# UCSD-Comp-Imaging/Nerf-Simple

Measured on AMD Instinct MI355X. Metric: ray-samples/sec at 800x800x128, higher is better.
Workload: dtype f16

## Files before the change

nerf-simple_amd/csrc/dw_gemm.hip:

```cpp
#include "nerf_device.h"
#include "launchers.h"

using namespace nerf_layout;

typedef __bf16 bf16x4 __attribute__((ext_vector_type(4)));

namespace {

constexpr int MAXD = 16;
struct GemmDesc {
    const __bf16* A;
    const __bf16* B;
    float* C;
    int lda, ldb, ldc;
    int M, N;
    int r0, Mv, Nv;
    int wg0, wgs;
    float* bias;
};
struct GemmTable {
    GemmDesc d[MAXD];
    int n;
    long long P;
};

constexpr int SLAB = 32;
static_assert(SLAB == 32, "the slab loop is written for two k-steps");
static_assert(ACT_TILE_PTS % SLAB == 0 && ACT_TILE_PTS * 16 == 4096, "a slab never straddles activation blocks");
constexpr int ROWB = 512;
constexpr int OPB = SLAB * ROWB;
constexpr int KSTEP = 16 * ROWB;
constexpr int SLOTB = 2 * OPB;
constexpr int RING = 4;
constexpr int LDS_BYTES = RING * SLOTB;
constexpr int DMA_PER_SLAB = 2 * SLAB / 2 / 8;

struct Frag { bf16x4 lo, hi; };
template <int KOFF>
__device__ __forceinline__ void read_frag_tr(Frag& f, unsigned addr_lo, unsigned addr_hi) {
    asm volatile("ds_read_b64_tr_b16 %0, %2 offset:%4\n\tds_read_b64_tr_b16 %1, %3 offset:%4"
                 : "=&v"(f.lo), "=&v"(f.hi) : "v"(addr_lo), "v"(addr_hi), "n"(KOFF));
}
__device__ __forceinline__ void frags_landed(Frag (&a)[4], Frag (&b)[2]) {
    asm volatile("s_waitcnt lgkmcnt(0)"
                 : "+v"(a[0].lo), "+v"(a[0].hi), "+v"(a[1].lo), "+v"(a[1].hi), "+v"(a[2].lo), "+v"(a[2].hi),
                   "+v"(a[3].lo), "+v"(a[3].hi), "+v"(b[0].lo), "+v"(b[0].hi), "+v"(b[1].lo), "+v"(b[1].hi));
}
__device__ __forceinline__ bf16x8 whole(const Frag& f) {
    return bf16x8{f.lo[0], f.lo[1], f.lo[2], f.lo[3], f.hi[0], f.hi[1], f.hi[2], f.hi[3]};
}

__global__ __launch_bounds__(512, 2) void dw_gemm_kernel(GemmTable tab) {
    extern __shared__ __attribute__((aligned(16))) char smem[];
    int di = 0;
    while (di + 1 < tab.n && (int)blockIdx.x >= tab.d[di + 1].wg0) ++di;
    const GemmDesc d = tab.d[di];
    const int slice = blockIdx.x - d.wg0;
    const long long nslab = (tab.P + SLAB - 1) / SLAB;
    const long long s_begin = nslab * slice / d.wgs, s_end = nslab * (slice + 1) / d.wgs;

    const int tid = threadIdx.x, lane = tid & 63;
    const int wave = __builtin_amdgcn_readfirstlane(tid >> 6);
    const int wm = wave >> 2, wn = wave & 3;
    const int m0 = 128 * wm, n0 = 64 * wn;

    const bool pieceA = wave < 4;
    const int pld = pieceA ? d.lda : d.ldb;
    const bool pblk = pld == 0;
    const __bf16* pbase = pieceA ? d.A : d.B;
    const int pwidth = pieceA ? d.M : d.N;
    const long long row_begin = s_begin * SLAB;
    const long long row_end = s_end * SLAB < tab.P ? s_end * SLAB : tab.P;
    const long long slice_rows = row_end > row_begin ? row_end - row_begin : 0;
    const long long slice_blocks = (row_end + ACT_TILE_PTS - 1) / ACT_TILE_PTS - row_begin / ACT_TILE_PTS;
    const __amdgpu_buffer_rsrc_t rs = pblk
        ? __builtin_amdgcn_make_buffer_rsrc(const_cast<char*>(reinterpret_cast<const char*>(pbase))
                                                + (row_begin / ACT_TILE_PTS) * ACT_BLOCK_BYTES,
                                            0, (int)(slice_rows > 0 ? slice_blocks * ACT_BLOCK_BYTES : 0), 0x00020000)
        : __builtin_amdgcn_make_buffer_rsrc(const_cast<__bf16*>(pbase + row_begin * pld), 0,
                                            (int)(slice_rows * pld * 2), 0x00020000);
    constexpr unsigned OUTSIDE = 0xffffffffu;
    unsigned voff[DMA_PER_SLAB];
    unsigned ldst[DMA_PER_SLAB];
    int vrow[DMA_PER_SLAB];
#pragma unroll
    for (int k = 0; k < DMA_PER_SLAB; ++k) {
        const int piece = wave * DMA_PER_SLAB + k, pi = piece & 15;
        ldst[k] = (piece >> 4) * OPB + pi * 1024;
        if (pblk) {
            const int c = 4 * (pi & 7) + (lane >> 4);
            vrow[k] = 16 * (pi >> 3) + ((lane & 15) ^ ((lane >> 4) << 2));
            voff[k] = c * 8 < pwidth ? (unsigned)(c * (ACT_TILE_PTS * 16) + vrow[k] * 16) : OUTSIDE;
        } else {
            vrow[k] = 2 * pi + (lane >> 5);
            const int cg = (lane & 31) ^ ((vrow[k] & 3) << 2);
            voff[k] = cg * 8 < pwidth ? (unsigned)(vrow[k] * pld * 2 + cg * 16) : OUTSIDE;
        }
    }
    auto issue_slab = [&](int it, int slot) {
        const long long p0 = row_begin + (long long)it * SLAB;
        unsigned vadd;
        int rows_left = SLAB;
        if (pblk) {
            vadd = (unsigned)((p0 / ACT_TILE_PTS - row_begin / ACT_TILE_PTS) * ACT_BLOCK_BYTES + (p0 % ACT_TILE_PTS) * 16);
            rows_left = tab.P - p0 < SLAB ? (int)(tab.P - p0) : SLAB;
        } else {
            vadd = (unsigned)it * (unsigned)(SLAB * pld * 2);
        }
#pragma unroll
        for (int k = 0; k < DMA_PER_SLAB; ++k) {
            lds_void* dst = reinterpret_cast<lds_void*>(reinterpret_cast<lds_char*>(0) + slot * SLOTB + ldst[k]);
            const unsigned off = (voff[k] == OUTSIDE || vrow[k] >= rows_left) ? OUTSIDE : voff[k] + vadd;
            __builtin_amdgcn_raw_ptr_buffer_load_lds(rs, dst, 16, off, 0, 0, 2);
        }
    };

    const int grp = lane >> 4, q = (lane & 15) >> 2, pp = lane & 3, h = lane >> 5;
    const int cl = 2 * (grp & 1) + (pp >> 1);
    auto frag_addr = [&](bool blocked, int t, int second) -> unsigned {
        const int r = 8 * h + q + 4 * second;
        if (blocked) return (4 * t + cl) * 256 + ((r ^ (cl << 2)) * 16) + 8 * (pp & 1);
        return r * ROWB + ((((4 * t + cl) ^ ((r & 3) << 2))) * 16) + 8 * (pp & 1);
    };
    unsigned aoff[4][2], boff[2][2];
#pragma unroll
    for (int i = 0; i < 4; ++i)
#pragma unroll
        for (int e = 0; e < 2; ++e) aoff[i][e] = frag_addr(d.lda == 0, m0 / 32 + i, e);
#pragma unroll
    for (int j = 0; j < 2; ++j)
#pragma unroll
        for (int e = 0; e < 2; ++e) boff[j][e] = OPB + frag_addr(d.ldb == 0, n0 / 32 + j, e);

    f32x16 acc[4][2];
#pragma unroll
    for (int i = 0; i < 4; ++i)
#pragma unroll
        for (int j = 0; j < 2; ++j)
#pragma unroll
            for (int r = 0; r < 16; ++r) acc[i][j][r] = 0.f;
    const bool active = m0 < d.M && n0 < d.N;
    float bsum[8] = {0.f, 0.f, 0.f, 0.f, 0.f, 0.f, 0.f, 0.f};
    const int brow = tid & 15, bchunk = tid >> 4;
    const unsigned baddr = bchunk * 256 + ((brow ^ ((bchunk & 3) << 2)) * 16);

#pragma unroll
    for (int k = 0; k < RING - 1; ++k)
        if (s_begin + k < s_end) issue_slab(k, k);
    Frag a0[4], b0[2], a1[4], b1[2];
    auto read_k0 = [&](unsigned base) {
#pragma unroll
        for (int i = 0; i < 4; ++i) read_frag_tr<0>(a0[i], base + aoff[i][0], base + aoff[i][1]);
#pragma unroll
        for (int j = 0; j < 2; ++j) read_frag_tr<0>(b0[j], base + boff[j][0], base + boff[j][1]);
    };
    if (s_begin < s_end) {
        const long long n = s_end - s_begin;
        if (n >= 3) asm volatile("s_waitcnt vmcnt(8)" ::: "memory");
        else if (n == 2) asm volatile("s_waitcnt vmcnt(4)" ::: "memory");
        else asm volatile("s_waitcnt vmcnt(0)" ::: "memory");
        __builtin_amdgcn_s_barrier();
        if (active) read_k0(0);
    }
    for (long long s = s_begin; s < s_end; ++s) {
        const int it = (int)(s - s_begin), slot = it & (RING - 1);
        const long long left = s_end - s;
        const unsigned base = slot * SLOTB;
        if (active) {
            frags_landed(a0, b0);
#pragma unroll
            for (int i = 0; i < 4; ++i) read_frag_tr<KSTEP>(a1[i], base + aoff[i][0], base + aoff[i][1]);
#pragma unroll
            for (int j = 0; j < 2; ++j) read_frag_tr<KSTEP>(b1[j], base + boff[j][0], base + boff[j][1]);
            __builtin_amdgcn_sched_barrier(0);
#pragma unroll
            for (int i = 0; i < 4; ++i)
#pragma unroll
                for (int j = 0; j < 2; ++j)
                    acc[i][j] = __builtin_amdgcn_mfma_f32_32x32x16_bf16(whole(a0[i]), whole(b0[j]), acc[i][j], 0, 0, 0);
            __builtin_amdgcn_sched_barrier(0);
        }
        if (left >= 2) {
            if (left >= 3) asm volatile("s_waitcnt vmcnt(4)" ::: "memory");
            else asm volatile("s_waitcnt vmcnt(0)" ::: "memory");
            __builtin_amdgcn_s_barrier();
            if (s + RING - 1 < s_end) issue_slab(it + RING - 1, (it + RING - 1) & (RING - 1));
        }
        if (active) {
            frags_landed(a1, b1);
            if (left >= 2) read_k0(((it + 1) & (RING - 1)) * SLOTB);
            __builtin_amdgcn_sched_barrier(0);
#pragma unroll
            for (int i = 0; i < 4; ++i)
#pragma unroll
                for (int j = 0; j < 2; ++j)
                    acc[i][j] = __builtin_amdgcn_mfma_f32_32x32x16_bf16(whole(a1[i]), whole(b1[j]), acc[i][j], 0, 0, 0);
        }
        if (d.bias && bchunk * 8 < d.M) {
#pragma unroll
            for (int ks = 0; ks < SLAB / 16; ++ks) {
                const bf16x8 v = *reinterpret_cast<const __attribute__((address_space(3))) bf16x8*>(
                    reinterpret_cast<lds_char*>(0) + base + ks * KSTEP + baddr);
#pragma unroll
                for (int k = 0; k < 8; ++k) bsum[k] += (float)v[k];
            }
        }
    }
    __syncthreads();
    if (d.bias && bchunk * 8 < d.M && s_begin < s_end) {
        float* red = reinterpret_cast<float*>(smem);
#pragma unroll
        for (int k = 0; k < 8; ++k) red[(brow * 32 + bchunk) * 8 + k] = bsum[k];
    }
    __syncthreads();
    if (d.bias && s_begin < s_end && tid < d.M) {
        const int ch = tid >> 3, k = tid & 7;
        float v = 0.f;
        for (int r = 0; r < 16; ++r) v += reinterpret_cast<float*>(smem)[(r * 32 + ch) * 8 + k];
        atomicAdd(d.bias + tid, v);
    }
    if (active && s_begin < s_end) {
#pragma unroll
        for (int i = 0; i < 4; ++i)
#pragma unroll
            for (int j = 0; j < 2; ++j)
#pragma unroll
                for (int r = 0; r < 16; ++r) {
                    const int row = m0 + 32 * i + (r & 3) + 8 * (r >> 2) + 4 * h - d.r0;
                    const int col = n0 + 32 * j + (lane & 31);
                    if (row >= 0 && row < d.Mv && col < d.Nv)
                        atomicAdd(d.C + (long long)row * d.ldc + col, acc[i][j][r]);
                }
    }
}

__global__ __launch_bounds__(256) void pack_draw_kernel(const float* __restrict__ d_raw, __bf16* __restrict__ dsr,
                                                        long long P, float* __restrict__ g_rgb_b,
                                                        float* __restrict__ g_sig_b) {
    __shared__ float red[4][4];
    f32x4 s = {0.f, 0.f, 0.f, 0.f};
    const __bf16 z = (__bf16)0.f;
    for (long long p = blockIdx.x * (long long)blockDim.x + threadIdx.x; p < P; p += (long long)gridDim.x * blockDim.x) {
        const f32x4 d = *reinterpret_cast<const f32x4*>(d_raw + p * 4);
        s += d;
        bf16x8* o = reinterpret_cast<bf16x8*>(dsr + p * 32);
        o[0] = bf16x8{(__bf16)d[0], (__bf16)d[1], (__bf16)d[2], (__bf16)d[3], z, z, z, z};
        o[1] = bf16x8{z, z, z, z, z, z, z, z};
        o[2] = o[1];
        o[3] = o[1];
    }
#pragma unroll
    for (int k = 0; k < 4; ++k) {
        float v = s[k];
#pragma unroll
        for (int off = 32; off >= 1; off >>= 1) v += __shfl_xor(v, off);
        if ((threadIdx.x & 63) == 0) red[threadIdx.x >> 6][k] = v;
    }
    __syncthreads();
    if (threadIdx.x < 4) {
        const float v = red[0][threadIdx.x] + red[1][threadIdx.x] + red[2][threadIdx.x] + red[3][threadIdx.x];
        atomicAdd(threadIdx.x < 3 ? g_rgb_b + threadIdx.x : g_sig_b, v);
    }
}

__global__ __launch_bounds__(256) void zero_f32_kernel(float* __restrict__ p, long long n) {
    const long long i = (blockIdx.x * (long long)blockDim.x + threadIdx.x) * 4;
    if (i + 3 < n) *reinterpret_cast<f32x4*>(p + i) = f32x4{0.f, 0.f, 0.f, 0.f};
    else for (long long k = i; k < n; ++k) p[k] = 0.f;
}

}

extern "C" int nerf_amd_launch_param_gradients_begin(const float* d_raw, void* scratch, float* grads, long long P,
                                                     hipStream_t stream) {
    (void)hipGetLastError();
    static_assert(PARAM_COUNT % 4 == 0, "16-byte zero fill");
    hipLaunchKernelGGL(zero_f32_kernel, dim3((PARAM_COUNT / 4 + 255) / 256), dim3(256), 0, stream, grads,
                       (long long)PARAM_COUNT);
    hipError_t e = hipGetLastError();
    if (e != hipSuccess) return (int)e;
    if (P <= 0) return 0;
    hipLaunchKernelGGL(pack_draw_kernel, dim3(512), dim3(256), 0, stream, d_raw, reinterpret_cast<__bf16*>(scratch), P,
                       grads + OFF_C1_B, grads + OFF_SIG_B);
    return (int)hipGetLastError();
}

extern "C" int nerf_amd_launch_param_gradients_finish(const void* acts_v, const void* dys_v, const void* posx64_v,
                                                      const void* posd32_v, const void* scratch, float* grads,
                                                      long long P, int bucket, hipStream_t stream) {
    (void)hipGetLastError();
    hipError_t e = hipSuccess;
    if (P <= 0) return 0;
    const __bf16* acts = reinterpret_cast<const __bf16*>(acts_v);
    const __bf16* dys = reinterpret_cast<const __bf16*>(dys_v);
    const __bf16* posx = reinterpret_cast<const __bf16*>(posx64_v);
    const __bf16* posd = reinterpret_cast<const __bf16*>(posd32_v);
    const __bf16* dsr = reinterpret_cast<const __bf16*>(scratch);
    auto act = [&](int L) { return acts + act_offset_bytes(L, P) / 2; };
    auto dy = [&](int L) { return dys + act_offset_bytes(L, P) / 2; };
    constexpr int BLK = 0;

    GemmTable t{};
    t.P = P;
    int n = 0;
    auto add = [&](const __bf16* A, int lda, int M, const __bf16* B, int ldb, int N, int coff, int ldc, int r0,
                   int Mv, int Nv, int boff = -1) {
        GemmDesc& g = t.d[n++];
        g.A = A; g.lda = lda; g.M = M; g.B = B; g.ldb = ldb; g.N = N;
        g.C = grads + coff; g.ldc = ldc; g.r0 = r0; g.Mv = Mv; g.Nv = Nv;
        g.bias = boff >= 0 ? grads + boff : nullptr;
    };
    const int LW = 256 * 256 + 256;
    add(dy(0), BLK, 256, posx, 64, 64, OFF_L0_W, 63, 0, 256, 63, OFF_L0_B);
    for (int l = 1; l <= 4; ++l)
        add(dy(l), BLK, 256, act(l - 1), BLK, 256, OFF_L1_W + (l - 1) * LW, 256, 0, 256, 256,
            OFF_L1_W + (l - 1) * LW + 65536);
    add(dy(5), BLK, 256, act(4), BLK, 256, OFF_SKIP_W, 319, 0, 256, 256, OFF_SKIP_B);
    add(dy(5), BLK, 256, posx, 64, 64, OFF_SKIP_W + 256, 319, 0, 256, 63);
    add(dy(6), BLK, 256, act(5), BLK, 256, OFF_L6_W, 256, 0, 256, 256, OFF_L6_W + 65536);
    add(dy(7), BLK, 256, act(6), BLK, 256, OFF_L6_W + LW, 256, 0, 256, 256, OFF_L6_W + LW + 65536);
    add(dsr, 32, 32, act(7), BLK, 256, OFF_SIG_W, 256, 3, 1, 256);
    add(dy(8), BLK, 256, act(7), BLK, 256, OFF_L2_W, 256, 0, 256, 256, OFF_L2_B);
    add(dy(9), BLK, 128, act(8), BLK, 256, OFF_C0_W, 283, 0, 128, 256, OFF_C0_B);
    add(dy(9), BLK, 128, posd, 32, 32, OFF_C0_W + 256, 283, 0, 128, 27);
    add(dsr, 32, 32, act(9), BLK, 128, OFF_C1_W, 128, 0, 3, 128);
    if (bucket != 0) {
        int m = 0;
        for (int i = 0; i < n; ++i) {
            const bool head = t.d[i].C - grads < GRAD_BUCKET_SPLIT;
            if (head == (bucket == 2)) t.d[m++] = t.d[i];
        }
        n = m;
    }
    t.n = n;
    constexpr double slab_cost = 1024.0;
    const int cus = device_cus();
    double total = 0;
    for (int i = 0; i < n; ++i) total += (double)(t.d[i].M + t.d[i].N) + slab_cost;
    const long long nslab = (P + SLAB - 1) / SLAB;
    const long long need = (P * 512 >> 30) + 1;
    long long w[16];
    double rem[16];
    long long used = 0;
    for (int i = 0; i < n; ++i) {
        const double share = ((double)(t.d[i].M + t.d[i].N) + slab_cost) / total * cus;
        w[i] = (long long)share;
        rem[i] = share - (double)w[i];
        if (w[i] < need) { w[i] = need; rem[i] = 0; }
        if (w[i] >= nslab) { w[i] = nslab; rem[i] = -1; }
        used += w[i];
    }
    while (used < cus) {
        int best = -1;
        for (int i = 0; i < n; ++i)
            if (rem[i] >= 0 && w[i] < nslab && (best < 0 || rem[i] > rem[best])) best = i;
        if (best < 0) break;
        ++w[best]; rem[best] = 0; ++used;
    }
    int wg = 0;
    for (int i = 0; i < n; ++i) {
        t.d[i].wg0 = wg;
        t.d[i].wgs = (int)w[i];
        wg += (int)w[i];
    }
    e = allow_dynamic_lds(reinterpret_cast<const void*>(dw_gemm_kernel), LDS_BYTES);
    if (e != hipSuccess) return (int)e;
    hipLaunchKernelGGL(dw_gemm_kernel, dim3(wg), dim3(512), LDS_BYTES, stream, t);

    return (int)hipGetLastError();
}

extern "C" int nerf_amd_launch_param_gradients(const float* d_raw, const void* acts_v, const void* dys_v,
                                               const void* posx64_v, const void* posd32_v, void* scratch,
                                               float* grads, long long P, hipStream_t stream) {
    const int rc = nerf_amd_launch_param_gradients_begin(d_raw, scratch, grads, P, stream);
    if (rc) return rc;
    return nerf_amd_launch_param_gradients_finish(acts_v, dys_v, posx64_v, posd32_v, scratch, grads, P, 0, stream);
}
```

Before: 1.405 billion.

## Fold narrow weight-gradient GEMMs as riders into host GEMMs sharing an operand

The two narrow weight-gradient GEMMs (sigma head from dsr, and the posd part of the colour layer) no longer get their own workgroup slices. Each rides on a host GEMM that streams the same activation operand, so that operand is read once. The rider tile is DMA'd into extra LDS per slot and accumulated in an extra MFMA accumulator, or by otherwise idle waves. The change also compacts the per-wave address registers, using XOR offsets and a reduced voff array, and templates the slab loop by role. In exchange it costs more LDS per slot, changes the vmcnt waits and the host-side weighting, and adds validity checks that could reject configurations.

```diff
diff --git a/nerf-simple_amd/csrc/dw_gemm.hip b/nerf-simple_amd/csrc/dw_gemm.hip
--- a/nerf-simple_amd/csrc/dw_gemm.hip
+++ b/nerf-simple_amd/csrc/dw_gemm.hip
@@ -17,6 +17,10 @@
     int r0, Mv, Nv;
     int wg0, wgs;
     float* bias;
+    const __bf16* R;
+    float* RC;
+    int rA;
+    int rldc, rr0, rMv, rNv;
 };
 struct GemmTable {
     GemmDesc d[MAXD];
@@ -30,9 +34,13 @@
 constexpr int ROWB = 512;
 constexpr int OPB = SLAB * ROWB;
 constexpr int KSTEP = 16 * ROWB;
-constexpr int SLOTB = 2 * OPB;
+constexpr int RIDW = 32;
+constexpr int RIDB = SLAB * RIDW * 2;
+constexpr int RKSTEP = 16 * RIDW * 2;
+constexpr int SLOTB = 2 * OPB + RIDB;
 constexpr int RING = 4;
-constexpr int LDS_BYTES = RING * SLOTB;
+constexpr int SPARE = RING * SLOTB;
+constexpr int LDS_BYTES = SPARE + 6 * 1024;
 constexpr int DMA_PER_SLAB = 2 * SLAB / 2 / 8;
 
 struct Frag { bf16x4 lo, hi; };
@@ -45,6 +53,28 @@
     asm volatile("s_waitcnt lgkmcnt(0)"
                  : "+v"(a[0].lo), "+v"(a[0].hi), "+v"(a[1].lo), "+v"(a[1].hi), "+v"(a[2].lo), "+v"(a[2].hi),
                    "+v"(a[3].lo), "+v"(a[3].hi), "+v"(b[0].lo), "+v"(b[0].hi), "+v"(b[1].lo), "+v"(b[1].hi));
+}
+enum { ROLE_HOST, ROLE_HOST_RIDER, ROLE_RIDER_B, ROLE_IDLE };
+template <int V> struct Role { static constexpr int value = V; };
+constexpr int ATILE = 4 * 256;
+template <int KOFF>
+__device__ __forceinline__ void read_a_tiles(Frag (&a)[4], unsigned addr_lo, unsigned addr_hi) {
+    read_frag_tr<KOFF>(a[0], addr_lo, addr_hi);
+    read_frag_tr<KOFF + ATILE>(a[1], addr_lo, addr_hi);
+    read_frag_tr<KOFF + 2 * ATILE>(a[2], addr_lo, addr_hi);
+    read_frag_tr<KOFF + 3 * ATILE>(a[3], addr_lo, addr_hi);
+}
+template <int KOFF>
+__device__ __forceinline__ void read_rider_now(Frag& f, unsigned addr) {
+    asm volatile("ds_read_b64_tr_b16 %0, %2 offset:%3\n\tds_read_b64_tr_b16 %1, %2 offset:%4\n\ts_waitcnt lgkmcnt(0)"
+                 : "=&v"(f.lo), "=&v"(f.hi) : "v"(addr), "n"(KOFF), "n"(KOFF + 4 * RIDW * 2));
+}
+template <int KOFF, int RKOFF>
+__device__ __forceinline__ void read_pair_now(Frag& a, Frag& f, unsigned addr_lo, unsigned addr_hi, unsigned addr) {
+    asm volatile("ds_read_b64_tr_b16 %0, %4 offset:%7\n\tds_read_b64_tr_b16 %1, %5 offset:%7\n\t"
+                 "ds_read_b64_tr_b16 %2, %6 offset:%8\n\tds_read_b64_tr_b16 %3, %6 offset:%9\n\ts_waitcnt lgkmcnt(0)"
+                 : "=&v"(a.lo), "=&v"(a.hi), "=&v"(f.lo), "=&v"(f.hi)
+                 : "v"(addr_lo), "v"(addr_hi), "v"(addr), "n"(KOFF), "n"(RKOFF), "n"(RKOFF + 4 * RIDW * 2));
 }
 __device__ __forceinline__ bf16x8 whole(const Frag& f) {
     return bf16x8{f.lo[0], f.lo[1], f.lo[2], f.lo[3], f.hi[0], f.hi[1], f.hi[2], f.hi[3]};
@@ -80,23 +110,28 @@
         : __builtin_amdgcn_make_buffer_rsrc(const_cast<__bf16*>(pbase + row_begin * pld), 0,
                                             (int)(slice_rows * pld * 2), 0x00020000);
     constexpr unsigned OUTSIDE = 0xffffffffu;
-    unsigned voff[DMA_PER_SLAB];
+    unsigned voff[2];
+    const unsigned pstep = pblk ? 8u * (ACT_TILE_PTS * 16) : 8u * (unsigned)pld;
     unsigned ldst[DMA_PER_SLAB];
-    int vrow[DMA_PER_SLAB];
+    const int prow = pblk ? 16 * ((wave & 3) >> 1) + ((lane & 15) ^ ((lane >> 4) << 2)) : 0;
 #pragma unroll
     for (int k = 0; k < DMA_PER_SLAB; ++k) {
         const int piece = wave * DMA_PER_SLAB + k, pi = piece & 15;
         ldst[k] = (piece >> 4) * OPB + pi * 1024;
+        if (k >= 2) continue;
         if (pblk) {
             const int c = 4 * (pi & 7) + (lane >> 4);
-            vrow[k] = 16 * (pi >> 3) + ((lane & 15) ^ ((lane >> 4) << 2));
-            voff[k] = c * 8 < pwidth ? (unsigned)(c * (ACT_TILE_PTS * 16) + vrow[k] * 16) : OUTSIDE;
+            voff[k] = (unsigned)(c * (ACT_TILE_PTS * 16) + prow * 16);
         } else {
-            vrow[k] = 2 * pi + (lane >> 5);
-            const int cg = (lane & 31) ^ ((vrow[k] & 3) << 2);
-            voff[k] = cg * 8 < pwidth ? (unsigned)(vrow[k] * pld * 2 + cg * 16) : OUTSIDE;
-        }
-    }
+            const int vrow = 2 * pi + (lane >> 5);
+            const int cg = (lane & 31) ^ ((vrow & 3) << 2);
+            voff[k] = cg * 8 < pwidth ? (unsigned)(vrow * pld * 2 + cg * 16) : OUTSIDE;
+        }
+    }
+    const int rider = d.R ? (d.rA ? 1 : 2) : 0;
+    const __amdgpu_buffer_rsrc_t rrs = __builtin_amdgcn_make_buffer_rsrc(
+        const_cast<__bf16*>(d.R + (rider ? row_begin * RIDW : 0)), 0, (int)(rider ? slice_rows * RIDW * 2 : 0), 0x00020000);
+    const unsigned rdst = wave < 2 ? 2 * OPB + wave * 1024 : SPARE + (wave - 2) * 1024;
     auto issue_slab = [&](int it, int slot) {
         const long long p0 = row_begin + (long long)it * SLAB;
         unsigned vadd;
@@ -110,8 +145,15 @@
 #pragma unroll
         for (int k = 0; k < DMA_PER_SLAB; ++k) {
             lds_void* dst = reinterpret_cast<lds_void*>(reinterpret_cast<lds_char*>(0) + slot * SLOTB + ldst[k]);
-            const unsigned off = (voff[k] == OUTSIDE || vrow[k] >= rows_left) ? OUTSIDE : voff[k] + vadd;
+            const bool beyond = pblk && 32 * (4 * (wave & 1) + k) >= pwidth;
+            const unsigned off = (beyond || voff[k & 1] == OUTSIDE || prow >= rows_left) ? OUTSIDE
+                                                                                         : voff[k & 1] + (vadd + (k >> 1) * pstep);
             __builtin_amdgcn_raw_ptr_buffer_load_lds(rs, dst, 16, off, 0, 0, 2);
+        }
+        if (rider) {
+            lds_void* dst = reinterpret_cast<lds_void*>(reinterpret_cast<lds_char*>(0) + (wave < 2 ? slot * SLOTB : 0) + rdst);
+            const unsigned off = wave < 2 ? (unsigned)it * (unsigned)RIDB + wave * 1024 + lane * 16 : OUTSIDE;
+            __builtin_amdgcn_raw_ptr_buffer_load_lds(rrs, dst, 16, off, 0, 0, 2);
         }
     };
 
@@ -122,24 +164,26 @@
         if (blocked) return (4 * t + cl) * 256 + ((r ^ (cl << 2)) * 16) + 8 * (pp & 1);
         return r * ROWB + ((((4 * t + cl) ^ ((r & 3) << 2))) * 16) + 8 * (pp & 1);
     };
-    unsigned aoff[4][2], boff[2][2];
+    const bool active = m0 < d.M && n0 < d.N;
+    const bool ride_a = rider == 1 && active;
+    const int bswap = ride_a ? wm : 0;
+    const bool ride_b = rider == 2 && !active && wm == 1 && 32 * wn < d.M;
+    const unsigned roff = 2 * OPB + (8 * h + q) * (RIDW * 2) + cl * 16 + 8 * (pp & 1);
+    const int at0 = ride_b ? wn : m0 / 32;
+    const unsigned aoff = frag_addr(d.lda == 0, at0, 0), boff = OPB + frag_addr(d.ldb == 0, n0 / 32 + bswap, 0);
+    unsigned ax = d.lda == 0 ? 64u : 2048u, bx = d.ldb == 0 ? 64u : 2048u, bt = d.ldb == 0 ? 1024u : 64u;
+    auto fresh = [&] { asm volatile("" : "+s"(ax), "+s"(bx), "+s"(bt)); };
+
+    f32x16 acc[4][2];
 #pragma unroll
     for (int i = 0; i < 4; ++i)
 #pragma unroll
-        for (int e = 0; e < 2; ++e) aoff[i][e] = frag_addr(d.lda == 0, m0 / 32 + i, e);
-#pragma unroll
-    for (int j = 0; j < 2; ++j)
-#pragma unroll
-        for (int e = 0; e < 2; ++e) boff[j][e] = OPB + frag_addr(d.ldb == 0, n0 / 32 + j, e);
-
-    f32x16 acc[4][2];
-#pragma unroll
-    for (int i = 0; i < 4; ++i)
-#pragma unroll
         for (int j = 0; j < 2; ++j)
 #pragma unroll
             for (int r = 0; r < 16; ++r) acc[i][j][r] = 0.f;
-    const bool active = m0 < d.M && n0 < d.N;
+    f32x16 racc;
+#pragma unroll
+    for (int r = 0; r < 16; ++r) racc[r] = 0.f;
     float bsum[8] = {0.f, 0.f, 0.f, 0.f, 0.f, 0.f, 0.f, 0.f};
     const int brow = tid & 15, bchunk = tid >> 4;
     const unsigned baddr = bchunk * 256 + ((brow ^ ((bchunk & 3) << 2)) * 16);
@@ -149,75 +193,107 @@
         if (s_begin + k < s_end) issue_slab(k, k);
     Frag a0[4], b0[2], a1[4], b1[2];
     auto read_k0 = [&](unsigned base) {
-#pragma unroll
-        for (int i = 0; i < 4; ++i) read_frag_tr<0>(a0[i], base + aoff[i][0], base + aoff[i][1]);
-#pragma unroll
-        for (int j = 0; j < 2; ++j) read_frag_tr<0>(b0[j], base + boff[j][0], base + boff[j][1]);
+        read_a_tiles<0>(a0, base + aoff, base + (aoff ^ ax));
+        read_frag_tr<0>(b0[0], base + boff, base + (boff ^ bx));
+        read_frag_tr<0>(b0[1], base + (boff ^ bt), base + (boff ^ bt ^ bx));
     };
     if (s_begin < s_end) {
         const long long n = s_end - s_begin;
-        if (n >= 3) asm volatile("s_waitcnt vmcnt(8)" ::: "memory");
-        else if (n == 2) asm volatile("s_waitcnt vmcnt(4)" ::: "memory");
-        else asm volatile("s_waitcnt vmcnt(0)" ::: "memory");
+        if (n >= 3) {
+            if (rider) asm volatile("s_waitcnt vmcnt(10)" ::: "memory");
+            else asm volatile("s_waitcnt vmcnt(8)" ::: "memory");
+        } else if (n == 2) {
+            if (rider) asm volatile("s_waitcnt vmcnt(5)" ::: "memory");
+            else asm volatile("s_waitcnt vmcnt(4)" ::: "memory");
+        } else asm volatile("s_waitcnt vmcnt(0)" ::: "memory");
         __builtin_amdgcn_s_barrier();
         if (active) read_k0(0);
     }
-    for (long long s = s_begin; s < s_end; ++s) {
-        const int it = (int)(s - s_begin), slot = it & (RING - 1);
-        const long long left = s_end - s;
-        const unsigned base = slot * SLOTB;
-        if (active) {
-            frags_landed(a0, b0);
-#pragma unroll
-            for (int i = 0; i < 4; ++i) read_frag_tr<KSTEP>(a1[i], base + aoff[i][0], base + aoff[i][1]);
-#pragma unroll
-            for (int j = 0; j < 2; ++j) read_frag_tr<KSTEP>(b1[j], base + boff[j][0], base + boff[j][1]);
-            __builtin_amdgcn_sched_barrier(0);
-#pragma unroll
-            for (int i = 0; i < 4; ++i)
-#pragma unroll
-                for (int j = 0; j < 2; ++j)
-                    acc[i][j] = __builtin_amdgcn_mfma_f32_32x32x16_bf16(whole(a0[i]), whole(b0[j]), acc[i][j], 0, 0, 0);
-            __builtin_amdgcn_sched_barrier(0);
-        }
-        if (left >= 2) {
-            if (left >= 3) asm volatile("s_waitcnt vmcnt(4)" ::: "memory");
-            else asm volatile("s_waitcnt vmcnt(0)" ::: "memory");
-            __builtin_amdgcn_s_barrier();
-            if (s + RING - 1 < s_end) issue_slab(it + RING - 1, (it + RING - 1) & (RING - 1));
-        }
-        if (active) {
-            frags_landed(a1, b1);
-            if (left >= 2) read_k0(((it + 1) & (RING - 1)) * SLOTB);
-            __builtin_amdgcn_sched_barrier(0);
-#pragma unroll
-            for (int i = 0; i < 4; ++i)
-#pragma unroll
-                for (int j = 0; j < 2; ++j)
-                    acc[i][j] = __builtin_amdgcn_mfma_f32_32x32x16_bf16(whole(a1[i]), whole(b1[j]), acc[i][j], 0, 0, 0);
-        }
-        if (d.bias && bchunk * 8 < d.M) {
-#pragma unroll
-            for (int ks = 0; ks < SLAB / 16; ++ks) {
-                const bf16x8 v = *reinterpret_cast<const __attribute__((address_space(3))) bf16x8*>(
-                    reinterpret_cast<lds_char*>(0) + base + ks * KSTEP + baddr);
-#pragma unroll
-                for (int k = 0; k < 8; ++k) bsum[k] += (float)v[k];
+    auto slab_loop = [&](auto role) {
+        constexpr int ROLE = decltype(role)::value;
+        constexpr bool HOST = ROLE == ROLE_HOST || ROLE == ROLE_HOST_RIDER;
+        for (long long s = s_begin; s < s_end; ++s) {
+            const int it = (int)(s - s_begin), slot = it & (RING - 1);
+            const long long left = s_end - s;
+            const unsigned base = slot * SLOTB;
+            fresh();
+            if constexpr (HOST) {
+                Frag rf;
+                if constexpr (ROLE == ROLE_HOST_RIDER) read_rider_now<0>(rf, base + roff);
+                frags_landed(a0, b0);
+                read_a_tiles<KSTEP>(a1, base + aoff, base + (aoff ^ ax));
+                read_frag_tr<KSTEP>(b1[0], base + boff, base + (boff ^ bx));
+                read_frag_tr<KSTEP>(b1[1], base + (boff ^ bt), base + (boff ^ bt ^ bx));
+                __builtin_amdgcn_sched_barrier(0);
+                if constexpr (ROLE == ROLE_HOST_RIDER)
+                    racc = __builtin_amdgcn_mfma_f32_32x32x16_bf16(whole(rf), whole(b0[0]), racc, 0, 0, 0);
+#pragma unroll
+                for (int i = 0; i < 4; ++i)
+#pragma unroll
+                    for (int j = 0; j < 2; ++j)
+                        acc[i][j] = __builtin_amdgcn_mfma_f32_32x32x16_bf16(whole(a0[i]), whole(b0[j]), acc[i][j], 0, 0, 0);
+                __builtin_amdgcn_sched_barrier(0);
+            } else if constexpr (ROLE == ROLE_RIDER_B) {
+                Frag ta, rf;
+                read_pair_now<0, 0>(ta, rf, base + aoff, base + (aoff ^ ax), base + roff);
+                acc[0][0] = __builtin_amdgcn_mfma_f32_32x32x16_bf16(whole(ta), whole(rf), acc[0][0], 0, 0, 0);
             }
-        }
-    }
+            if (left >= 2) {
+                if (left >= 3) {
+                    if (rider) asm volatile("s_waitcnt vmcnt(5)" ::: "memory");
+                    else asm volatile("s_waitcnt vmcnt(4)" ::: "memory");
+                } else asm volatile("s_waitcnt vmcnt(0)" ::: "memory");
+                __builtin_amdgcn_s_barrier();
+                if (s + RING - 1 < s_end) issue_slab(it + RING - 1, (it + RING - 1) & (RING - 1));
+            }
+            if constexpr (HOST) {
+                Frag rf;
+                if constexpr (ROLE == ROLE_HOST_RIDER) read_rider_now<RKSTEP>(rf, base + roff);
+                frags_landed(a1, b1);
+                if (left >= 2) read_k0(((it + 1) & (RING - 1)) * SLOTB);
+                __builtin_amdgcn_sched_barrier(0);
+                if constexpr (ROLE == ROLE_HOST_RIDER)
+                    racc = __builtin_amdgcn_mfma_f32_32x32x16_bf16(whole(rf), whole(b1[0]), racc, 0, 0, 0);
+#pragma unroll
+                for (int i = 0; i < 4; ++i)
+#pragma unroll
+                    for (int j = 0; j < 2; ++j)
+                        acc[i][j] = __builtin_amdgcn_mfma_f32_32x32x16_bf16(whole(a1[i]), whole(b1[j]), acc[i][j], 0, 0, 0);
+            } else if constexpr (ROLE == ROLE_RIDER_B) {
+                Frag ta, rf;
+                read_pair_now<KSTEP, RKSTEP>(ta, rf, base + aoff, base + (aoff ^ ax), base + roff);
+                acc[0][0] = __builtin_amdgcn_mfma_f32_32x32x16_bf16(whole(ta), whole(rf), acc[0][0], 0, 0, 0);
+            }
+            if (d.bias && bchunk * 8 < d.M) {
+#pragma unroll
+                for (int ks = 0; ks < SLAB / 16; ++ks) {
+                    const bf16x8 v = *reinterpret_cast<const __attribute__((address_space(3))) bf16x8*>(
+                        reinterpret_cast<lds_char*>(0) + base + ks * KSTEP + baddr);
+#pragma unroll
+                    for (int k = 0; k < 8; ++k) bsum[k] += (float)v[k];
+                }
+            }
+        }
+    };
+    if (ride_a) slab_loop(Role<ROLE_HOST_RIDER>{});
+    else if (active) slab_loop(Role<ROLE_HOST>{});
+    else if (ride_b) slab_loop(Role<ROLE_RIDER_B>{});
+    else slab_loop(Role<ROLE_IDLE>{});
     __syncthreads();
-    if (d.bias && bchunk * 8 < d.M && s_begin < s_end) {
+    int etid = tid;
+    asm volatile("" : "+v"(etid));
+    const int elane = etid & 63, eh = elane >> 5, ebrow = etid & 15, ebchunk = etid >> 4;
+    if (d.bias && ebchunk * 8 < d.M && s_begin < s_end) {
         float* red = reinterpret_cast<float*>(smem);
 #pragma unroll
-        for (int k = 0; k < 8; ++k) red[(brow * 32 + bchunk) * 8 + k] = bsum[k];
+        for (int k = 0; k < 8; ++k) red[(ebrow * 32 + ebchunk) * 8 + k] = bsum[k];
     }
     __syncthreads();
-    if (d.bias && s_begin < s_end && tid < d.M) {
-        const int ch = tid >> 3, k = tid & 7;
+    if (d.bias && s_begin < s_end && etid < d.M) {
+        const int ch = etid >> 3, k = etid & 7;
         float v = 0.f;
         for (int r = 0; r < 16; ++r) v += reinterpret_cast<float*>(smem)[(r * 32 + ch) * 8 + k];
-        atomicAdd(d.bias + tid, v);
+        atomicAdd(d.bias + etid, v);
     }
     if (active && s_begin < s_end) {
 #pragma unroll
@@ -226,11 +302,21 @@
             for (int j = 0; j < 2; ++j)
 #pragma unroll
                 for (int r = 0; r < 16; ++r) {
-                    const int row = m0 + 32 * i + (r & 3) + 8 * (r >> 2) + 4 * h - d.r0;
-                    const int col = n0 + 32 * j + (lane & 31);
+                    const int row = m0 + 32 * i + (r & 3) + 8 * (r >> 2) + 4 * eh - d.r0;
+                    const int col = n0 + 32 * (j ^ bswap) + (elane & 31);
                     if (row >= 0 && row < d.Mv && col < d.Nv)
                         atomicAdd(d.C + (long long)row * d.ldc + col, acc[i][j][r]);
                 }
+    }
+    if ((ride_a || ride_b) && s_begin < s_end) {
+        const int rrow0 = ride_b ? 32 * wn : 0, rcol0 = ride_b ? 0 : n0 + 32 * wm;
+#pragma unroll
+        for (int r = 0; r < 16; ++r) {
+            const int row = rrow0 + (r & 3) + 8 * (r >> 2) + 4 * eh - d.rr0;
+            const int col = rcol0 + (elane & 31);
+            if (row >= 0 && row < d.rMv && col < d.rNv)
+                atomicAdd(d.RC + (long long)row * d.rldc + col, ride_b ? acc[0][0][r] : racc[r]);
+        }
     }
 }
 
@@ -310,6 +396,12 @@
         g.C = grads + coff; g.ldc = ldc; g.r0 = r0; g.Mv = Mv; g.Nv = Nv;
         g.bias = boff >= 0 ? grads + boff : nullptr;
     };
+    auto ride = [&](const __bf16* R, bool for_A, int coff, int ldc, int r0, int Mv, int Nv) {
+        GemmDesc& g = t.d[n - 1];
+        g.R = R; g.rA = for_A; g.RC = grads + coff; g.rldc = ldc; g.rr0 = r0; g.rMv = Mv; g.rNv = Nv;
+    };
+    static_assert(OFF_SIG_W >= GRAD_BUCKET_SPLIT && OFF_L2_W >= GRAD_BUCKET_SPLIT && OFF_C0_W >= GRAD_BUCKET_SPLIT,
+                  "both riders and their hosts are in the late bucket");
     const int LW = 256 * 256 + 256;
     add(dy(0), BLK, 256, posx, 64, 64, OFF_L0_W, 63, 0, 256, 63, OFF_L0_B);
     for (int l = 1; l <= 4; ++l)
@@ -319,10 +411,10 @@
     add(dy(5), BLK, 256, posx, 64, 64, OFF_SKIP_W + 256, 319, 0, 256, 63);
     add(dy(6), BLK, 256, act(5), BLK, 256, OFF_L6_W, 256, 0, 256, 256, OFF_L6_W + 65536);
     add(dy(7), BLK, 256, act(6), BLK, 256, OFF_L6_W + LW, 256, 0, 256, 256, OFF_L6_W + LW + 65536);
-    add(dsr, 32, 32, act(7), BLK, 256, OFF_SIG_W, 256, 3, 1, 256);
     add(dy(8), BLK, 256, act(7), BLK, 256, OFF_L2_W, 256, 0, 256, 256, OFF_L2_B);
+    ride(dsr, true, OFF_SIG_W, 256, 3, 1, 256);
     add(dy(9), BLK, 128, act(8), BLK, 256, OFF_C0_W, 283, 0, 128, 256, OFF_C0_B);
-    add(dy(9), BLK, 128, posd, 32, 32, OFF_C0_W + 256, 283, 0, 128, 27);
+    ride(posd, false, OFF_C0_W + 256, 283, 0, 128, 27);
     add(dsr, 32, 32, act(9), BLK, 128, OFF_C1_W, 128, 0, 3, 128);
     if (bucket != 0) {
         int m = 0;
@@ -333,17 +425,27 @@
         n = m;
     }
     t.n = n;
+    for (int i = 0; i < n; ++i) {
+        const GemmDesc& g = t.d[i];
+        bool ok = g.lda == 0 || g.M <= 32;
+        if (g.R) {
+            ok = ok && (g.rA ? g.M == 256 && g.N == 256 : g.lda == 0 && g.M <= 128 && g.N == 256);
+            ok = ok && (g.C - grads < GRAD_BUCKET_SPLIT) == (g.RC - grads < GRAD_BUCKET_SPLIT);
+        }
+        if (!ok) return (int)hipErrorInvalidValue;
+    }
     constexpr double slab_cost = 1024.0;
     const int cus = device_cus();
+    auto weight = [&](const GemmDesc& g) { return (double)(g.M + g.N + (g.R ? RIDW : 0)) + slab_cost; };
     double total = 0;
-    for (int i = 0; i < n; ++i) total += (double)(t.d[i].M + t.d[i].N) + slab_cost;
+    for (int i = 0; i < n; ++i) total += weight(t.d[i]);
     const long long nslab = (P + SLAB - 1) / SLAB;
     const long long need = (P * 512 >> 30) + 1;
     long long w[16];
     double rem[16];
     long long used = 0;
     for (int i = 0; i < n; ++i) {
-        const double share = ((double)(t.d[i].M + t.d[i].N) + slab_cost) / total * cus;
+        const double share = weight(t.d[i]) / total * cus;
         w[i] = (long long)share;
         rem[i] = share - (double)w[i];
         if (w[i] < need) { w[i] = need; rem[i] = 0; }
```

Result: no change. 1.404 billion (-0.0%).
